# yijingru/KG_Instance_Segmentation

Measured on AMD Instinct MI355X. Metric: imgs/s (train fwd+bwd) at 512x512, higher is better.
Workload: dtype forward: f32-tolerance, hi + lo f16 planes (22 significant bits), 3 MFMA products / backward: f16 single planes, 1 MFMA product; f16 MFMA, fp32 accumulate; 1 GPU; KGnet train step fwd(dec+seg)+4xDetectionLossAll+SEG_loss+bwd+Adam, batch 8/GPU 3x512x512, 300 boxes/img, full HIP path; precision_policy=fp32, global_batch=8, parallelism=dp1, loss_readback=every step (train.py:156), grad_overflow=False

## Files before the change

### kg_instance_segmentation_amd/csrc/norm_pool.hip

```cpp
#include "kg_common.h"

struct RowsR { const bf16_t* p; int ld, P, ps; };
struct RowsW { bf16_t* p; int ld, P, ps; };
__device__ __forceinline__ void rd8(const RowsR& t, long r, int c, float (&v)[8]) { kg_load_planes8(t.p + r * t.ld + c, t.P, t.ps, v); }
__device__ __forceinline__ void wr8(const RowsW& t, long r, int c, float (&v)[8]) { kg_store_planes<8>(t.p + r * t.ld + c, t.P, t.ps, v, true); }
#define KG_PLANES(pl)                                                       \
    const kg_planes_t pp = kg_planes_or_default(pl);                        \
    KG_CHECK_ARG(kg_planes_ok(pp), "bad kg_planes_t (at most 3 planes, strides multiples of 8)")

__global__ void img_pack_kernel(const float* __restrict__ img, RowsW out, int N, int C, int HW) {
    long total = (long)N * HW;
    for (long i = blockIdx.x * (long)blockDim.x + threadIdx.x; i < total; i += (long)gridDim.x * blockDim.x) {
        long n = i / HW, p = i - n * HW;
        float v[8];
#pragma unroll
        for (int c = 0; c < 8; ++c) v[c] = c < C ? img[(n * C + c) * HW + p] : 0.f;
        wr8(out, i, 0, v);
    }
}
extern "C" int kg_img_pack(const float* img, void* out, int ldout, int N, int C, int H, int W, const kg_planes_t* planes, void* stream) {
    KG_CHECK_ARG(img && out && C <= 8 && ldout >= 8 && ldout % 8 == 0, "kg_img_pack: bad args");
    KG_PLANES(planes);
    long total = (long)N * H * W;
    int blocks = (int)((total + 255) / 256); if (blocks > 8192) blocks = 8192;
// ... 526 lines not shown
        }
        const float sy = (float)ih / (float)oh, sx = (float)iw / (float)ow;
        int ylo, yhi, xlo, xhi;
        bil_cand(iy, sy, oh, &ylo, &yhi); bil_cand(ix, sx, ow, &xlo, &xhi);
        float g[8];
#pragma unroll
        for (int e = 0; e < 8; ++e) g[e] = 0.f;
        for (int oy = ylo; oy <= yhi; ++oy) {
            int y0, y1; float ly;
            bil_src(oy, sy, ih, &y0, &y1, &ly);
            float wy = (y0 == iy ? 1.f - ly : 0.f) + (y1 == iy ? ly : 0.f);
            if (y0 != iy && y1 != iy) continue;
            for (int ox = xlo; ox <= xhi; ++ox) {
                int x0, x1; float lx;
                bil_src(ox, sx, iw, &x0, &x1, &lx);
                if (x0 != ix && x1 != ix) continue;
                float wx = (x0 == ix ? 1.f - lx : 0.f) + (x1 == ix ? lx : 0.f);
                float w = wy * wx;
                float ds[8];
                rd8(dy, out0 + (long)oy * ow + ox, c, ds);
#pragma unroll
                for (int e = 0; e < 8; ++e) g[e] += w * ds[e];
            }
        }
        if (mask) {
            const uint4 mv = *reinterpret_cast<const uint4*>(mask + p * ldmask + c);
            const bf16_t* ms = reinterpret_cast<const bf16_t*>(&mv);
#pragma unroll
            for (int e = 0; e < 8; ++e) g[e] = bf2f(ms[e]) > 0.f ? g[e] : 0.f;
        }
        wr8(dx, p, c, g);
    }
}
extern "C" int kg_bilinear_fwd(const void* x, int ldx, void* y, int ldy, int N, int IH, int IW, int OH, int OW, int C,
                               const int* boxdesc, const int* row2box, long total_out_rows, const kg_planes_t* planes, void* stream) {
    KG_CHECK_ARG(x && y && C % 8 == 0 && ldx % 8 == 0 && ldy % 8 == 0, "kg_bilinear_fwd: bad args");
    KG_PLANES(planes);
    long rows = boxdesc ? total_out_rows : (long)N * OH * OW;
    if (rows == 0) return KG_OK;
    long total = rows * (C / 8);
    static const int fast2x = getenv("KG_BILINEAR_2X") ? atoi(getenv("KG_BILINEAR_2X")) : 1;
    if (fast2x && !boxdesc && OH == 2 * IH && OW == 2 * IW && IH >= 2 && IW >= 2) {
        const long threads = (long)N * ((IH + BIL2_ROWS - 1) / BIL2_ROWS) * IW * (C / 8);
        int blocks2 = (int)((threads + 255) / 256); if (blocks2 > 65536) blocks2 = 65536;
        hipLaunchKernelGGL(bilinear2x_fwd_kernel, dim3(blocks2), dim3(256), 0, (hipStream_t)stream, RowsR{(const bf16_t*)x, ldx, pp.a_planes, pp.a_pstride},
                           RowsW{(bf16_t*)y, ldy, pp.y_planes, pp.y_pstride}, N, IH, IW, C / 8);
        KG_CHECK_LAUNCH("bilinear2x_fwd");
        return KG_OK;
    }
    int blocks = (int)((total + 255) / 256); if (blocks > 16384) blocks = 16384;
    hipLaunchKernelGGL(bilinear_fwd_kernel, dim3(blocks), dim3(256), 0, (hipStream_t)stream, RowsR{(const bf16_t*)x, ldx, pp.a_planes, pp.a_pstride},
                       RowsW{(bf16_t*)y, ldy, pp.y_planes, pp.y_pstride}, IH, IW, OH, OW, C / 8, rows, (const BilBox*)boxdesc, row2box);
    KG_CHECK_LAUNCH("bilinear_fwd");
    return KG_OK;
}
extern "C" int kg_bilinear_bwd(const void* dy, int lddy, void* dx, int lddx, int N, int IH, int IW, int OH, int OW, int C,
                               const int* boxdesc, const int* row2box, long total_in_rows, const void* mask, int ldmask,
                               const kg_planes_t* planes, void* stream) {
    KG_CHECK_ARG(dy && dx && C % 8 == 0 && lddy % 8 == 0 && lddx % 8 == 0 && (!mask || ldmask % 8 == 0), "kg_bilinear_bwd: bad args");
    KG_PLANES(planes);
    long rows = boxdesc ? total_in_rows : (long)N * IH * IW;
    if (rows == 0) return KG_OK;
    long total = rows * (C / 8);
    int blocks = (int)((total + 255) / 256); if (blocks > 16384) blocks = 16384;
    hipLaunchKernelGGL(bilinear_bwd_kernel, dim3(blocks), dim3(256), 0, (hipStream_t)stream, RowsR{(const bf16_t*)dy, lddy, pp.a_planes, pp.a_pstride},
                       RowsW{(bf16_t*)dx, lddx, pp.y_planes, pp.y_pstride}, IH, IW, OH, OW, C / 8, rows, (const BilBox*)boxdesc, row2box, (const bf16_t*)mask, ldmask);
    KG_CHECK_LAUNCH("bilinear_bwd");
    return KG_OK;
}

__global__ void add_rows_kernel(const RowsR a, const RowsR b,
                                const bf16_t* __restrict__ m, int ldm, const RowsW y, long M, int C8, const float* __restrict__ sc,
                                const float* __restrict__ sc2) {
    long total = M * C8;
    const float s = sc ? *sc * (sc2 ? *sc2 : 1.f) : 1.f;
    for (long i = blockIdx.x * (long)blockDim.x + threadIdx.x; i < total; i += (long)gridDim.x * blockDim.x) {
        long r; int c; kg_divmod(i, C8, &r, &c); c *= 8;
        float v[8];
        rd8(a, r, c, v);
        if (b.p) {
            float bs[8];
            rd8(b, r, c, bs);
#pragma unroll
            for (int e = 0; e < 8; ++e) v[e] += bs[e];
        }
        if (s != 1.f) {
#pragma unroll
            for (int e = 0; e < 8; ++e) v[e] *= s;
        }
        if (m) {
            uint4 mv = *reinterpret_cast<const uint4*>(m + r * ldm + c);
            const bf16_t* ms = (const bf16_t*)&mv;
#pragma unroll
            for (int e = 0; e < 8; ++e) v[e] = bf2f(ms[e]) > 0.f ? v[e] : 0.f;
        }
        wr8(y, r, c, v);
// ... 156 lines not shown
```

### kg_instance_segmentation_amd/csrc/conv_halo.hip

```cpp
#include "conv_args.h"
#include <type_traits>
#include <utility>
#include <stdlib.h>
#ifndef KG_HALO_SETPRIO
#define KG_HALO_SETPRIO 0
#endif
#ifndef KG_NARROW_V2
#define KG_NARROW_V2 1
#endif

__device__ uint4 kg_halo_zero_line[8];

struct HaloArgs {
    const bf16_t* x; const bf16_t* w; const float* bias;
    bf16_t* y; float* y_f32; const bf16_t* res; const bf16_t* mask;
    const int4* tiletab;
    int ntiles;
    int N, H, W, tiles_x, tiles_y;
    int cin_pad, ldx, Cout, ldy, ldres, ldmask, K, flip, relu, f32_C, f32_hw;
    int grp_chunks; const int* vmap; float* f32_b; float* f32_c;
    int xcd_map;
    int head_split;
    KMap km; int grp_C;
    float* stat_part;
    KgBStat bs;
    int kp_raw;
    int yP, yps, rP, rps;
    int walk3;
    const float* oscale;
    int prod_split; float* part;
    int ksplit; float* kpart;
    int nb2;
};

static void halo_set_walk(HaloArgs& a, int xP, int wP) {
    int xi[6], wj[6];
    const int nv = kg_plane_pairs(xP, wP, xi, wj);
    constexpr int on = 1;
    a.walk3 = on && nv == 3 && xi[0] == 0 && xi[1] == 1 && xi[2] == 0;
}

template <int KS, int WC, int WPX, int GM = 0, bool BSK = false>
__global__ __launch_bounds__(WC * WPX * 64) void conv_halo_kernel(const HaloArgs a) {
    constexpr int KSX = GM == 3 ? 1 : (GM == 4 ? 2 : KS);
    constexpr int PAD = KS / 2, TW = 4 * WPX, HWD = TW + KS - 1, HPIX = (16 + KS - 1) * HWD, TC = WC * 64, NT = WC * WPX * 64, T = KS * KSX;
    static_assert(GM < 3 || KS == 7, "the narrow variants are written for 7 x 7 kernels");
    constexpr int HALO_BYTES = HPIX * 128, WBUF_BYTES = TC * 128;
    constexpr bool GLW = KS == 7 && WC <= 2;
    constexpr int NSL = GLW ? 6 : 3;
    constexpr bool ASMRD = GLW && GM != 1;
    constexpr int WPT = TC * 8 / NT;
    extern __shared__ __attribute__((aligned(16))) unsigned char smem[];
    unsigned char* halo = smem;
    unsigned char* wbuf = smem + HALO_BYTES;

    const int tid = threadIdx.x, lane = tid & 63, wave = tid >> 6;
    const int wc = wave / WPX, wp = wave % WPX;
    const int lm = lane & 15, g = lane >> 4;
    int oy0, ox0, Hd, Wd;
    long rowbase;
    int bix = blockIdx.x, biy = blockIdx.y;
    if (a.xcd_map) {
        const int L = blockIdx.y * gridDim.x + blockIdx.x;
        const int xcd = L & 7, slot = L >> 3;
        biy = slot % gridDim.y;
        bix = xcd * (gridDim.x >> 3) + slot / gridDim.y;
    }
    if (a.tiletab) {
        const int4 tt = a.tiletab[bix];
        rowbase = tt.x; Hd = tt.y >> 16; Wd = tt.y & 0xffff; oy0 = tt.z >> 16; ox0 = tt.z & 0xffff;
    } else {
        int bt = bix;
        const int tx = bt % a.tiles_x; bt /= a.tiles_x;
        const int ty = bt % a.tiles_y; const int n = bt / a.tiles_y;
        oy0 = ty * 16; ox0 = tx * TW; Hd = a.H; Wd = a.W; rowbase = (long)n * a.H * a.W;
    }
    const int c0 = GM == 1 ? 0 : biy * TC;

    f32x4 acc[4][4];
#pragma unroll
    for (int i = 0; i < 4; ++i)
#pragma unroll
        for (int j = 0; j < 4; ++j) acc[i][j] = f32x4{0.f, 0.f, 0.f, 0.f};

    int a_off[4][2];
#pragma unroll
    for (int i = 0; i < 4; ++i) {
        const int r = wc * 64 + (lm >> 2) * 16 + i * 4 + (lm & 3);
        const int key = 2 * ((r >> 4) & 3) + ((r >> 1) & 1);
#pragma unroll
        for (int s = 0; s < 2; ++s) a_off[i][s] = r * 128 + (((4 * s + g) ^ key) * 16);
    }
    const int xb = (wp >> 2) * 16 + lm;
    int kb[KS][2];
#pragma unroll
    for (int kx = 0; kx < KS; ++kx) {
        if constexpr (GM >= 3) {
            if (kx < KSX) {
#pragma unroll
                for (int s = 0; s < 2; ++s) {
                    int kcol = GM == 3 ? 4 * s + g : 4 * kx + 2 * s + (g >> 1);
                    if (kcol > KS - 1) kcol = KS - 1;
                    const int slot = GM == 3 ? 0 : 1 + (g & 1);
                    const int fx = a.flip ? KS - 1 - kcol : kcol;
                    kb[kx][s] = (((wp & 3) * 4) * HWD + xb + fx) * 128 + ((slot ^ ((xb + fx) & 6)) * 16);
                }
            } else kb[kx][0] = kb[kx][1] = 0;
            continue;
        }
        const int fx = a.flip ? KS - 1 - kx : kx;
        const int key = (xb + fx) & 6;
#pragma unroll
        for (int s = 0; s < 2; ++s) kb[kx][s] = (((wp & 3) * 4) * HWD + xb) * 128 + (((4 * s + g) ^ key) * 16);
    }
    int ab[NSL][2];
#pragma unroll
    for (int q = 0; q < NSL; ++q)
#pragma unroll
        for (int s = 0; s < 2; ++s) ab[q][s] = q * WBUF_BYTES + a_off[0][s];

    int w_row[WPT], w_lds[WPT];
#pragma unroll
    for (int i = 0; i < WPT; ++i) {
        int e = tid + i * NT, r = e >> 3, c = e & 7;
        w_row[i] = r;
        w_lds[i] = r * 128 + ((c ^ (2 * ((r >> 4) & 3) + ((r >> 1) & 1))) * 16);
    }
    const int wc8 = (tid & 7) * 8;
    uint4 wreg[WPT];

    auto mma = [&](auto mk, const bf16x8 (&af)[4], const bf16x8 (&bfr)[4]) {
        constexpr int MK = decltype(mk)::value;
        if (KG_HALO_SETPRIO) __builtin_amdgcn_s_setprio(1);
#pragma unroll
        for (int i = 0; i < 4; ++i)
            if ((MK >> i) & 1) {
// ... 35 lines not shown
        else xo = a.km.xoff(cc);
        if (!stage) {
        } else if (KS == 3) {
            constexpr int HPT = (HPIX * 8 + NT - 1) / NT;
            uint4 hreg[HPT];
#pragma unroll
            for (int q = 0; q < HPT; ++q) {
                const int e = tid + q * NT;
                const int p = e >> 3, c = e & 7;
                const int hy = p / HWD, hx = p - hy * HWD;
                const int iy = oy0 + hy - PAD, ix = ox0 + hx - PAD;
                uint4 v = make_uint4(0, 0, 0, 0);
                if (e < HPIX * 8 && (unsigned)iy < (unsigned)Hd && (unsigned)ix < (unsigned)Wd)
                    v = *reinterpret_cast<const uint4*>(a.x + (rowbase + (long)iy * Wd + ix) * a.ldx + xo + c * 8);
                hreg[q] = v;
            }
#pragma unroll
            for (int q = 0; q < HPT; ++q) {
                const int e = tid + q * NT;
                const int p = e >> 3, c = e & 7;
                const int hx = p % HWD;
                if (e < HPIX * 8) *reinterpret_cast<uint4*>(halo + p * 128 + ((c ^ (hx & 6)) * 16)) = hreg[q];
            }
        } else
        {
            constexpr int HPT = (HPIX * 8 + NT - 1) / NT;
            const int wave_u = __builtin_amdgcn_readfirstlane(wave);
#pragma unroll 1
            for (int q = 0; q < HPT; ++q) {
                const int e = tid + q * NT;
                if (e < HPIX * 8) {
                    const int p = e >> 3, cs = e & 7;
                    const int hy = p / HWD, hx = p - hy * HWD;
                    const int c = cs ^ (hx & 6);
                    const int iy = oy0 + hy - PAD, ix = ox0 + hx - PAD;
                    const bf16_t* src = reinterpret_cast<const bf16_t*>(kg_halo_zero_line) + c * 8;
                    if ((unsigned)iy < (unsigned)Hd && (unsigned)ix < (unsigned)Wd)
                        src = a.x + (rowbase + (long)iy * Wd + ix) * a.ldx + xo + c * 8;
                    __builtin_amdgcn_global_load_lds((const __attribute__((address_space(1))) void*)src,
                                                     (__attribute__((address_space(3))) void*)(halo + (q * NT + wave_u * 64) * 16), 16, 0, 0);
                }
            }
        }
        if constexpr (GM == 1) {
            const int head_n = cc / a.grp_chunks;
            if (head_n < 2) {
                constexpr int ROWB = 7 * 2048;
                const int wave_n = __builtin_amdgcn_readfirstlane(wave);
#if KG_NARROW_V2
                const bf16_t* nsrc[2];
#pragma unroll
                for (int k = 0; k < 2; ++k) {
                    const int e = tid + k * 512, kyl = e >> 7, rho = (e >> 3) & 15, sl = e & 7;
                    const int r = 16 * (rho >> 2) + 4 * head_n + (rho & 3);
                    const int key = 2 * (rho >> 2) + ((rho >> 1) & 1);
                    nsrc[k] = a.w + (long)r * a.K + (long)(kyl * KS) * a.cin_pad + cc * 64 + ((sl ^ key) * 8);
                }
                auto nload = [&](int kx) {
                    unsigned char* dst = wbuf + (kx % 3) * ROWB + wave_n * 1024;
                    const long ro = (long)kx * a.cin_pad;
                    __builtin_amdgcn_global_load_lds((const __attribute__((address_space(1))) void*)(nsrc[0] + ro),
                                                     (__attribute__((address_space(3))) void*)dst, 16, 0, 0);
                    if (wave_n < 6)
                        __builtin_amdgcn_global_load_lds((const __attribute__((address_space(1))) void*)(nsrc[1] + ro),
                                                         (__attribute__((address_space(3))) void*)(dst + 8192), 16, 0, 0);
                };
                nload(0); nload(1);
// ... 128 lines not shown
#pragma unroll
            for (int i = 0; i < WPT; ++i) *reinterpret_cast<uint4*>(wbuf + slot_bytes + w_lds[i]) = wreg[i];
        };
        const bf16_t* wsrc[WPT];
        auto wglds = [&](int slot_bytes) {
#pragma unroll
            for (int i = 0; i < WPT; ++i) {
                __builtin_amdgcn_global_load_lds((const __attribute__((address_space(1))) void*)wsrc[i],
                                                 (__attribute__((address_space(3))) void*)(wbuf + slot_bytes + (i * NT + __builtin_amdgcn_readfirstlane(wave) * 64) * 16), 16, 0, 0);
                wsrc[i] += a.cin_pad;
            }
        };
        auto wait_newest = [&]() {
            if constexpr (WPT == 1) asm volatile("s_waitcnt vmcnt(1)" ::: "memory");
            else asm volatile("s_waitcnt vmcnt(2)" ::: "memory");
        };
        static_assert(!GLW || WPT <= 2, "counted waits are written for 1 or 2 loads per slice");
        if constexpr (GLW) {
#pragma unroll
            for (int i = 0; i < WPT; ++i) {
                const int e = tid + i * NT, r = e >> 3, cs = e & 7;
                wsrc[i] = a.w + (long)(c0 + r) * a.K + cc * 64 + (cs ^ (2 * ((r >> 4) & 3) + ((r >> 1) & 1))) * 8;
            }
            wglds(0); wglds(WBUF_BYTES); wglds(2 * WBUF_BYTES); wglds(3 * WBUF_BYTES);
            wait_newest();
            __builtin_amdgcn_s_barrier();
            asm volatile("" ::: "memory");
        } else {
            wload(0); wstore(0);
            if (T > 1) { wload(1); wstore(1); }
            if (T > 2) wload(2);
            __syncthreads();
        }
        bf16x8 a0[4], b0[4], a1[4], b1[4];
        if constexpr (ASMRD) {
#pragma unroll
            for (int i = 0; i < 4; ++i) { a0[i] = bf16x8{0, 0, 0, 0, 0, 0, 0, 0}; a1[i] = a0[i]; }
        }
        const unsigned lds0 = lds_addr(smem);
        int abr[NSL][2];
        int sbr[NSL];
#pragma unroll
        for (int q = 0; q < NSL; ++q) { abr[q][0] = ab[q][0]; abr[q][1] = ab[q][1]; sbr[q] = q * WBUF_BYTES; }
        int tapb = a.flip ? ((KS - 1) * HWD + (GM >= 3 ? 0 : KS - 1)) * 128 : 0;
        const int sx = a.flip ? -128 : 128, sy = a.flip ? -HWD * 128 : HWD * 128;
        auto ldA = [&](auto mk, bf16x8 (&af)[4], int base) {
            constexpr int MK = decltype(mk)::value;
            if constexpr (ASMRD) {
                const unsigned ad = lds0 + HALO_BYTES + base;
                if (MK & 1) lds_rd128<0>(af[0], ad);
                if (MK & 2) lds_rd128<512>(af[1], ad);
                if (MK & 4) lds_rd128<1024>(af[2], ad);
                if (MK & 8) lds_rd128<1536>(af[3], ad);
            } else {
#pragma unroll
                for (int i = 0; i < 4; ++i)
                    if ((MK >> i) & 1) af[i] = *reinterpret_cast<const bf16x8*>(wbuf + base + i * 512);
            }
        };
        auto ldB = [&](bf16x8 (&bfr)[4], int tb, int kbv) {
            if constexpr (ASMRD) {
                const unsigned ad = lds0 + tb + kbv;
                lds_rd128<0>(bfr[0], ad); lds_rd128<HWD * 128>(bfr[1], ad); lds_rd128<2 * HWD * 128>(bfr[2], ad); lds_rd128<3 * HWD * 128>(bfr[3], ad);
            } else {
                const unsigned char* hb = halo + tb + kbv;
#pragma unroll
// ... 581 lines not shown
        }
    }
    if (!bsk) {
        hipLaunchKernelGGL((conv_halo_kernel<KS, WC, WPX, GM>), grid, dim3(WC * WPX * 64), smem, st, a);
        KG_KNAME(kname, "conv_halo_kernel<%d, %d, %d, %d>", KS, WC, WPX, GM);
        kg_note_kernel(kname);
    }
    KG_CHECK_LAUNCH("conv_halo");
    if (a.ksplit > 1) {
        hipLaunchKernelGGL((conv_halo_finish_kernel<WC, WPX>), dim3(grid.x, grid.y), dim3(WC * WPX * 64), 0, st, a);
        KG_CHECK_LAUNCH("conv_halo_finish");
    }
    return KG_OK;
}

extern "C" int kg_conv2d_halo(const void* x, const void* w, const float* bias, void* y, float* y_f32, const void* res,
                              const void* mask, int N, int H, int W, int cin_pad, int ldx, int Cout, int ldy, int ldres,
                              int ldmask, int K, int KS, int flip, int relu, int f32_C, int wc, const int* tiletab,
                              int ntiles, int total_rows, const kg_planes_t* planes, void* stream) {
    HaloArgs a;
    memset(&a, 0, sizeof(a));
    const kg_planes_t pp = kg_planes_or_default(planes);
    KG_CHECK_ARG(kg_planes_ok(pp), "kg_conv2d_halo: bad kg_planes_t");
    int segs_[3];
    const int vplanes = kg_kmap_segs(pp.a_planes, pp.w_planes, segs_);
    a.km = kg_make_kmap(cin_pad, 64, pp.a_planes, pp.a_pstride, pp.w_planes);
    halo_set_walk(a, pp.a_planes, pp.w_planes);
    a.yP = pp.y_planes; a.yps = pp.y_pstride; a.rP = pp.b_planes; a.rps = pp.b_pstride; a.oscale = pp.oscale;
    KG_CHECK_ARG(!(y_f32 && (res || mask)), "kg_conv2d_halo: fp32 exports take no residual / mask");
    KG_CHECK_ARG(x && w && (y || y_f32), "kg_conv2d_halo: null pointer");
    KG_CHECK_ARG(KS == 3 || KS == 7, "kg_conv2d_halo: kernel size must be 3 or 7");
    KG_CHECK_ARG(cin_pad % 64 == 0 && ldx % 8 == 0, "kg_conv2d_halo: cin_pad must be a multiple of 64 (got %d)", cin_pad);
    const int narrow = (wc >> 9) & 3;
    KG_CHECK_ARG(narrow == 0 || (narrow <= 2 && KS == 7 && cin_pad == 64 && vplanes == 1 && (wc & 255) <= 1 && !tiletab && y && !y_f32),
                 "kg_conv2d_halo: the narrow variants take one 64-channel single-plane dense input and a rows output");
    KG_CHECK_ARG(K >= (narrow ? 7 * narrow * 64 : KS * KS * cin_pad * vplanes), "kg_conv2d_halo: K too small");
    KG_CHECK_ARG((tiletab && ntiles > 0 && Cout > 0) || (N > 0 && H > 0 && W > 0 && Cout > 0), "kg_conv2d_halo: empty problem");
    a.x = (const bf16_t*)x; a.w = (const bf16_t*)w; a.bias = bias; a.y = (bf16_t*)y; a.y_f32 = y_f32;
    a.res = (const bf16_t*)res; a.mask = (const bf16_t*)mask;
    a.N = N; a.H = H; a.W = W; a.tiles_x = kg_cdiv(W, 16); a.tiles_y = kg_cdiv(H, 16);
    a.cin_pad = cin_pad * vplanes; a.ldx = ldx; a.Cout = Cout; a.ldy = ldy; a.ldres = ldres; a.ldmask = ldmask; a.K = K;
    a.flip = flip; a.relu = relu; a.f32_C = f32_C; a.tiletab = (const int4*)tiletab; a.ntiles = ntiles; a.f32_hw = total_rows;
    {
        const KgConvStats& cs = kg_conv_stats();
        const bool want = cs.bs.x ? (flip && KS == 3 && wc <= 1 && !tiletab && Cout % 64 == 0) : (!res && !mask && !relu && !flip);
        if (y && !y_f32 && want && cs.part && cs.nb == 0)
            a.stat_part = cs.part;
    }
    const int k1skip = (wc >> 8) & 1; wc &= 255;
    if (wc == 0) wc = 1;
    hipStream_t st = (hipStream_t)stream;
    if (KS == 7) {
        switch (wc) {
            case 1:
                if (narrow == 1) return launch_halo<7, 1, 8, 3>(a, st);
                if (narrow == 2) return launch_halo<7, 1, 8, 4>(a, st);
                return k1skip ? launch_halo<7, 1, 8, 2>(a, st) : launch_halo<7, 1, 8>(a, st);
            case 2: return launch_halo<7, 2, 4>(a, st);
            case 3: return launch_halo<7, 3, 4>(a, st);
        }
    } else {
        switch (wc) {
            case 1: return launch_halo<3, 1, 8>(a, st);
            case 2: return launch_halo<3, 2, 4>(a, st);
            case 3: return launch_halo<3, 3, 4>(a, st);
        }
    }
    kg_set_error("kg_conv2d_halo: bad wc %d", wc);
    return KG_ERR_ARG;
}

__global__ __launch_bounds__(256) void heads2_finish_kernel(const float* __restrict__ part, long per_z, int Z, int N, long hw, float* __restrict__ kp,
                                                            float* __restrict__ sh, float* __restrict__ md, int kp_raw) {
    for (long i = (long)blockIdx.x * 256 + threadIdx.x; i < per_z; i += (long)gridDim.x * 256) {
        double acc = 0.;
        for (int z = 0; z < Z; ++z) acc += (double)part[z * per_z + i];
        const float v = (float)acc;
        const long pix = i % hw, q = i / hw;
        const int ch = (int)(q % 55); const long n = q / 55;
        if (ch < 5) kp[(n * 5 + ch) * hw + pix] = kp_raw ? v : 1.f / (1.f + expf(-v));
        else if (ch < 15) sh[(n * 10 + ch - 5) * hw + pix] = v;
        else md[(n * 40 + ch - 15) * hw + pix] = v;
    }
}

extern "C" int kg_conv2d_halo_heads2(const void* x, const void* w, const float* bias64, const int* vmap, float* kp, float* sh,
                                     float* md, int N, int H, int W, int C, int ldx, int K, int kp_sigmoid, const kg_planes_t* planes, void* stream) {
    HaloArgs a;
    memset(&a, 0, sizeof(a));
// ... 68 lines not shown
```

### kg_instance_segmentation_amd/engine.py

```python
import os

import torch

from . import arch, ops
from .ops import BF16, PT, PackedWeight

PRECISIONS = {
    "fp32": (2, 2, 2, 2, 1),
    "fp32b2": (2, 2, 2, 2, 2),
    "half": (1, 1, 1, 1, 1),
    "halfmix": (2, 1, 1, 1, 1),
    "fp32bf": (3, 3, 3, 3, 2),
    "fp32bf_full": (3, 3, 3, 3, 3),
    "fp32bf_w1d1": (3, 3, 3, 3, 2, 1, 1),
    "fp32bf_b1": (3, 3, 3, 3, 1),
    "trunk2": (2, 2, 1, 1, 1), "mixed": (2, 1, 1, 1, 1), "bf16": (1, 1, 1, 1, 1),
}
HALF_POLICIES = ("fp32", "fp32b2", "half", "halfmix")
DEFAULT_PRECISION = "fp32"
PRE = [0]
NARROW_HEADS_DGRAD = int(os.environ.get("KG_NARROW_HEADS_DGRAD", "2"))
BN_BWD_STATS = True


def default_precision():
    p = os.environ.get("KG_PRECISION", DEFAULT_PRECISION)
    if p not in PRECISIONS:
        raise ValueError(f"KG_PRECISION must be one of {sorted(PRECISIONS)} (got {p!r})")
    return p


def trunc(t, P):
    if isinstance(t, PT):
        return t if t.P <= P else PT(t.t, P, t.ps)
    return t


class Var:
    __slots__ = ("t", "C", "relu", "grad", "masked", "pending", "pmasked", "req", "parent", "c0", "gP", "bn_part", "boundary", "gsc",
                 "uses", "ngot", "bn_in", "bstat")
    ENG = None

    def __init__(self, t, C, relu=False, req=True, parent=None, c0=0, gP=None):
        self.t = t if isinstance(t, PT) else PT(t)
        self.C, self.relu, self.req = C, relu, req
        self.gP = self.t.P if gP is None else gP
        self.grad, self.masked = None, True
        self.pending, self.pmasked = None, True
        self.parent, self.c0 = parent, c0
        self.boundary = False
        self.uses, self.ngot = 0, 0
        self.bn_in = None
        self.bstat = None
        self.gsc = None
# ... 588 lines not shown
        self._phase("end")
        if self.nbt:
            torch._foreach_add_(self.nbt, 1)
            self.nbt = []
        if self.stats_written:
            ops.PARAM_EPOCH[0] += 1
        self.feats, self.dims, self.N, self.maps = feats, dims, N, maps
        for fv in feats:
            fv.uses += 1 << 20
        feats[1].boundary = True
        return maps, feats, dims

    HEAD_OFF = (0, 8, 24)
    HEAD_PAD = (8, 16, 40)

    def heads2_tables(self, dev):
        t = getattr(self, "_heads2", None)
        if t is None or t["vmap"].device != dev:
            rows, vmap = ops.heads2_layout()
            vm = torch.tensor(vmap, dtype=torch.int32)
            t = {"rows": [torch.tensor(r, dtype=torch.int32, device=dev) for r in rows], "vmap": vm.to(dev),
                 "bias_idx": torch.where(vm < 0, torch.full_like(vm, 55), vm).long().to(dev),
                 "zero1": torch.zeros(1, dtype=torch.float32, device=dev)}
            self._heads2 = t
        return t

    def prepare_heads2(self, lvl, C, dev, train):
        self.heads2_seen[lvl] = (C, dev)
        key = f"heads_c{lvl}.2F"
        ent = self.fusedT.get(key)
        if self.fast_stamp is not None and ent is not None and ent[0][:3] == self.fast_stamp and ent[1].buf.device == dev:
            entT = self.fusedT.get(f"heads_c{lvl}.2T") if train else None
            if not train or (entT is not None and entT[0][:3] == self.fast_stamp and entT[1].buf.device == dev):
                return ent[1], ent[2], (entT[1], entT[2]) if train else None
        ph = self.ph
        specs = [self.spec(f"{h}_head_c{lvl}.2", C, co, 7, 1, 3, P=ph) for h, co in arch.HEADS]
        ws = [self.P(s.names[0] + ".weight") for s in specs]
        bs = [self.P(s.names[0] + ".bias") for s in specs]
        ver = self.stamp + tuple(t._version for t in ws + bs) + tuple(t.data_ptr() for t in ws + bs)
        if ent is None or ent[0] != ver or ent[1].buf.device != dev:
            lay = self.heads2_tables(dev)
            pwF = ent[1] if ent is not None and ent[1].buf.device == dev else PackedWeight(64, 49, C, dev, xP=ph, wP=ph, groups=3, dtype=self.dt)
            for k, w in enumerate(ws):
                pwF.pack_rows(w.detach(), lay["rows"][k], group=k)
            bias64 = torch.cat([b.detach() for b in bs] + [lay["zero1"]])[lay["bias_idx"]]
            self.fusedT[key] = (ver, pwF, bias64)
        _, pwF, bias64 = self.fusedT[key]
        pwT = None
        if train:
            key = f"heads_c{lvl}.2T"
            ent = self.fusedT.get(key)
            ver = self.stamp + tuple(w._version for w in ws) + tuple(w.data_ptr() for w in ws)
            if ent is None or ent[0] != ver or ent[1].buf.device != dev:
                gph = min(ph, self.pg)
                reuse = ent is not None and ent[1].buf.device == dev
                pwT = ent[1] if reuse else PackedWeight(3 * C, 49, 64, dev, xP=gph, wP=min(gph, self.pdw), dtype=self.dt)
                narrow = NARROW_HEADS_DGRAD and gph == 1 and min(gph, self.pdw) == 1
                pwN = None
                if narrow:
                    pwN = ent[2] if reuse and ent[2] is not None else (PackedWeight(C, 7, 64, dev, dtype=self.dt), PackedWeight(C, 14, 64, dev, dtype=self.dt))
                    pwN[0].pack_narrow(ws[0].detach(), 8)
                    pwN[1].pack_narrow(ws[1].detach(), 16)
                for k, w in enumerate(ws):
                    if narrow and k < 2:
                        continue
                    pwT.pack(w.detach(), row0=k * C, c0=self.HEAD_OFF[k], transposed=True)
                self.fusedT[key] = (ver, pwT, pwN)
            pwT = (self.fusedT[key][1], self.fusedT[key][2])
        return pwF, bias64, pwT

    def heads_second(self, hid, lvl, C, N, H, W):
        dev = hid.t.device
        train = self.tape is not None
        specs = [self.spec(f"{h}_head_c{lvl}.2", C, co, 7, 1, 3, P=self.ph) for h, co in arch.HEADS]
        pwF, bias64, pwTN = self.prepare_heads2(lvl, C, dev, train)
        pwT, pwN = pwTN if pwTN is not None else (None, None)
        outs = [torch.empty(N, co, H, W, dtype=torch.float32, device=dev) for _, co in arch.HEADS]
        ops.conv_halo_heads2(hid.t, pwF, bias64, self.heads2_tables(dev)["vmap"], outs[0], outs[1], outs[2], N, H, W, C,
                             kp_sigmoid=not self.raw_kp_logits)
        if self.keep_kp_logits:
            side = [torch.empty_like(o) for o in outs]
            ops.conv_halo_heads2(hid.t, pwF, bias64, self.heads2_tables(dev)["vmap"], side[0], side[1], side[2], N, H, W, C, kp_sigmoid=False)
            self.kp_logits[lvl] = side[0]
        slot = {"grad": None}
        self.head_slots.append((slot, lvl, N, H, W))
        wreq = [train and self.trainable((s.names[0] + ".weight", s.names[0] + ".bias")) for s in specs]
        if train and (hid.req or any(wreq)):
            geom = (N * H * W, H, W, H, W, 7, 7, 1, 3)

            def bwd():
                g = slot["grad"]
                if g is None:
                    return
                for k, ((h, co), s) in enumerate(zip(arch.HEADS, specs)):
                    if not wreq[k]:
                        continue
                    gk = g.cols(self.HEAD_OFF[k], self.HEAD_OFF[k] + self.HEAD_PAD[k])
                    w = self.P(s.names[0] + ".weight")
                    gw = self.new_grad(s.names[0] + ".weight", w)
                    db = self.new_grad(s.names[0] + ".bias", self.P(s.names[0] + ".bias"))
                    ops.conv_wgrad(trunc(hid.t, min(hid.gP, self.pw)).cols(k * C, (k + 1) * C), trunc(gk, self.pw), C, co, geom, [(gw, 0, co)], N=N, bias_out=db)
                    self.param_grads[s.names[0] + ".weight"] = gw
                    self.param_grads[s.names[0] + ".bias"] = db
                if not hid.req:
                    return
                dh = ops.alloc_pt(hid.rows, 3 * C, hid.gP, dev, dtype=self.dt)
                if pwN is not None and g.P == 1 and NARROW_HEADS_DGRAD >= 2 and dh.P == 1:
                    ops.conv7_narrow(g, pwN[0], C, N, H, W, dh.cols(0, C), mask=hid.t.hi()[:, :C], chan_lo=0, chan_slot=8, algo_cin=5)
                    ops.conv7_narrow(g, pwN[1], C, N, H, W, dh.cols(C, 2 * C), mask=hid.t.hi()[:, C:2 * C], chan_lo=8, chan_slot=16, algo_cin=10)
                elif pwN is not None and g.P == 1:
                    ops.conv_halo(g, pwN[0], C, N, H, W, 7, y=dh.cols(0, C), mask=hid.t.hi()[:, :C], flip=True, narrow=8, algo_cin=5)
                    ops.conv_halo(g, pwN[1], C, N, H, W, 7, y=dh.cols(C, 2 * C), mask=hid.t.hi()[:, C:2 * C], flip=True, narrow=16, algo_cin=10)
                else:
                    ops.conv_halo(g, pwT, 2 * C, N, H, W, 7, y=dh.cols(0, 2 * C), mask=hid.t.hi()[:, :2 * C], flip=True, k1skip=True, algo_cin=7.5)
                ops.conv_halo(g, pwT.rows_from(2 * C), C, N, H, W, 7, y=dh.cols(2 * C, 3 * C), mask=hid.t.hi()[:, 2 * C:], flip=True, algo_cin=40)
                hid.add_grad(dh, masked=True)
            self.tape.append(bwd)
        return outs

    def export_feats(self):
        outs = []
        for fv, (h, w) in zip(self.feats, self.dims):
            o = torch.empty(fv.rows, fv.C, dtype=torch.float32, device=fv.t.device)
            ops.planes_to_f32(fv.t, fv.C, o)
            outs.append(o.view(self.N, h, w, fv.C).permute(0, 3, 1, 2))
        return outs

    def backward_dec(self, map_grads, feat_grads, gscale=None):
        if gscale is not None:
            self.gscale = gscale
            Var.ENG = self
        gsc = self.gscale[0:1] if self.gscale is not None else None
        if self.grad_store is not None:
            self.grad_store.dense_backward_started()
        for (slot, lvl, N, Hh, Wh) in self.head_slots:
            gs = map_grads[3 * lvl:3 * lvl + 3]
            if all(g is None for g in gs):
                continue
            dev = self.maps[3 * lvl].device
            packed = ops.alloc_pt(N * Hh * Wh, 64, min(self.ph, self.pg), dev, dtype=self.dt)
            if all(g is not None for g in gs) and self.HEAD_OFF == (0, 8, 24) and sum(self.HEAD_PAD) == 64:
                ops.grad_pack3([g.contiguous().float() for g in gs], self.maps[3 * lvl], packed, N, [co for _, co in arch.HEADS], Hh, Wh, self.HEAD_PAD, scale=gsc)
                slot["grad"] = packed
                continue
            for k, g in enumerate(gs):
                co = arch.HEADS[k][1]
                view = packed.cols(self.HEAD_OFF[k], self.HEAD_OFF[k] + self.HEAD_PAD[k])
                if g is None:
# ... 50 lines not shown
```

### kg_instance_segmentation_amd/ops.py

```python
import functools
import math
import os

import torch

from . import _lib
from ._lib import c_int, c_long, c_float, c_double, ptr, stream_ptr

BF16 = torch.bfloat16
F16 = torch.float16
_scratch = {}
PARAM_EPOCH = [0]


def scratch_f32(nfloats, dev, tag="default"):
    key = (str(dev), tag)
    t = _scratch.get(key)
    if t is None or t.numel() < nfloats:
        t = torch.empty(max(int(nfloats), 1 << 16), dtype=torch.float32, device=dev)
        _scratch[key] = t
    return t


class WgradReduceQueue:
# ... 246 lines not shown
    if PACKQ16.jobs:
        PACKQ16.flush(hold)


def launch_held_packs():
    if PACKQ.pending is not None:
        PACKQ.launch_pending()
    if PACKQ16.pending is not None:
        PACKQ16.launch_pending()


class PackedWeight:

    def __init__(self, rows, taps, cin_pad, dev, xP=1, wP=1, groups=1, dtype=BF16):
        self.rows, self.taps, self.cin_pad, self.xP, self.wP, self.groups = rows, taps, cin_pad, xP, wP, groups
        self.vp = vplanes(xP, wP)
        self.tap_stride = groups * self.vp * cin_pad
        self.K = round_up((round_up(taps, 4) if cin_pad == 8 else taps) * self.tap_stride, 64)
        self.buf = torch.zeros(round_up(rows, 384), self.K, dtype=dtype, device=dev)

    def pack(self, w, row0=0, c0=0, transposed=False):
        Cout, Cin, KH, KW = w.shape
        assert w.dtype == torch.float32 and w.is_contiguous()
        assert self.groups == 1
        if PACKQ.defer:
            (PACKQ16 if fmt_of(self) else PACKQ).add(w, self, row0, c0, transposed, None)
            return
        _lib.call("kg_pack_weight", ptr(w), ptr(self.buf), Cout, Cin, KH, KW, self.K, self.cin_pad, row0, c0,
                  1 if transposed else 0, self.xP, self.wP, stream_ptr(), fmt=fmt_of(self))


    def pack_narrow(self, w, chan_slot, row0=0):
        Cout, Cin, KH, KW = w.shape
        assert w.dtype == torch.float32 and w.is_contiguous() and KH == KW == 7 and Cout <= chan_slot and self.xP == self.wP == 1
        assert self.cin_pad == 64 and self.K >= 7 * 8 * chan_slot
        if PACKQ.defer:
            (PACKQ16 if fmt_of(self) else PACKQ).add(w, self, row0, 0, True, None, tap_stride=chan_slot, tap_pitch=8, cin_pad=chan_slot)
            return
        _lib.call("kg_pack_weight_narrow", ptr(w), ptr(self.buf), Cout, Cin, KH, KW, self.K, row0, 0, chan_slot, 8, stream_ptr(), fmt=fmt_of(self))

    def rows_from(self, r0):
        v = PackedWeight.__new__(PackedWeight)
        v.rows, v.taps, v.cin_pad, v.K, v.buf = self.rows - r0, self.taps, self.cin_pad, self.K, self.buf[r0:]
        v.xP, v.wP, v.groups, v.vp, v.tap_stride = self.xP, self.wP, self.groups, self.vp, self.tap_stride
        return v

    def pack_rows(self, w, rowmap, group=0):
        Cout, Cin, KH, KW = w.shape
        assert w.dtype == torch.float32 and w.is_contiguous() and rowmap.dtype == torch.int32 and rowmap.numel() == Cout
        c0 = group * self.vp * self.cin_pad
        if PACKQ.defer:
            (PACKQ16 if fmt_of(self) else PACKQ).add(w, self, 0, c0, False, rowmap, self.tap_stride)
            return
        _lib.call("kg_pack_weight_rows", ptr(w), ptr(self.buf), Cout, Cin, KH, KW, self.K, self.cin_pad, ptr(rowmap), c0,
                  self.xP, self.wP, self.tap_stride, stream_ptr(), fmt=fmt_of(self))


def heads2_layout():
    grp = [[16 * q + 4 * i + r for q in range(4) for r in range(4)] for i in range(4)]
    rows = [grp[0][:5], grp[1][:10], grp[2] + grp[3] + grp[0][5:13]]
    vmap = [-1] * 64
    base = (0, 5, 15)
    for h in range(3):
        for c, v in enumerate(rows[h]):
            vmap[v] = base[h] + c
    return rows, vmap

# ... 35 lines not shown
IM2COL_WGRAD = True


HALO_WC = 0


USE_WS = True


def conv_halo(x, pw, cout, N, H, W, KS, y=None, y_f32=None, bias=None, res=None, mask=None, relu=False, flip=False, wc=0,
              tiletab=None, total_rows=0, k1skip=False, algo_cin=None, tiletab16=None, oscale=None, tiletab8=None, narrow=0):
    flush_packs()
    assert nplanes(x)[0] == pw.xP, (nplanes(x), pw.xP)
    if (USE_WS and KS == 3 and pw.cin_pad == 64 and cout == 64 and pw.xP == 2 and pw.wP == 2 and y is not None and y_f32 is None and res is None
            and mask is None and not flip and oscale is None and wc == 0 and HALO_WC == 0 and (tiletab is None or tiletab8 is not None)
            and nplanes(y)[0] <= 2 and not conv_stats_armed()):
        _lib.call("kg_conv3x3_ws", ptr(_rows(x)), ptr(pw.buf), ptr(bias), ptr(base(y)), N, H, W, ld(x), ld(y), pw.K, 1 if relu else 0,
                  ptr(tiletab8), tiletab8.shape[0] if tiletab8 is not None else 0, pl(a=x, y=y, w=pw.wP), stream_ptr(), fmt=fmt_of(x))
        return
    planes = pl(a=x, b=res, y=y, w=pw.wP, oscale=oscale)
    x, y, res, mask = base(x), base(y), base(res), base(mask)
    if (USE_C3 and planes is None and KS == 3 and pw.cin_pad == 64 and y is not None and y_f32 is None and wc == 0 and HALO_WC == 0
            and (tiletab is None or tiletab16 is not None)):
        flush_packs()
        _lib.call("kg_conv3x3_c64", ptr(_rows(x)), ptr(pw.buf), ptr(bias), ptr(y), ptr(res), ptr(mask), N, H, W, ld(x), cout, ld(y),
                  ld(res) if res is not None else 0, ld(mask) if mask is not None else 0, pw.K, 1 if flip else 0, 1 if relu else 0,
                  ptr(tiletab16), tiletab16.shape[0] if tiletab16 is not None else 0, stream_ptr(), fmt=fmt_of(x))
        return
    wc = wc or HALO_WC
    if k1skip:
        assert KS == 7 and wc in (0, 1)
        wc = 1 | 256
    if narrow:
        assert KS == 7 and wc in (0, 1) and flip and narrow in (8, 16) and planes is None and tiletab is None and y is not None and y_f32 is None
        wc = 1 | (512 if narrow == 8 else 1024)
    f32_C = 0
    if y_f32 is not None:
        f32_C = y_f32.shape[1] if y_f32.dim() == 4 else 1
    _lib.call("kg_conv2d_halo", ptr(_rows(x)), ptr(pw.buf), ptr(bias), ptr(y), ptr(y_f32), ptr(res), ptr(mask), N, H, W,
              pw.cin_pad, ld(x), cout, ld(y) if y is not None else 0, ld(res) if res is not None else 0,
              ld(mask) if mask is not None else 0, pw.K, KS, 1 if flip else 0, 1 if relu else 0, f32_C, wc, ptr(tiletab),
              tiletab.shape[0] if tiletab is not None else 0, total_rows, planes, stream_ptr(), fmt=fmt_of(x))


USE_1X1 = True
GATHER_1X1 = True


def conv1x1(x, pw, cout, y, bias=None, res=None, mask=None, relu=False):
    flush_packs()
    assert pw.vp == 1 and all(nplanes(t)[0] == 1 for t in (x, y, res))
    x, y, res, mask = base(x), base(y), base(res), base(mask)
    _lib.call("kg_conv1x1", ptr(_rows(x)), ptr(pw.buf), ptr(bias), ptr(_rows(y)), ptr(res), ptr(mask), c_long(x.shape[0]),
              pw.cin_pad, pw.K, ld(x), cout, ld(y), ld(res) if res is not None else 0, ld(mask) if mask is not None else 0,
              1 if relu else 0, stream_ptr(), fmt=fmt_of(x))


def can_1x1(x, pw, KH, stride, pad, y, y_f32, res=None):
    if pw.vp > 1 or any(nplanes(t)[0] > 1 for t in (x, y, res)):
        return False
    if GATHER_1X1 and pw.cin_pad >= 192 and pw.rows > 64:
        return False
    return (USE_1X1 and KH == 1 and stride == 1 and pad == 0 and y is not None and y_f32 is None and pw.cin_pad % 64 == 0
            and 64 <= pw.cin_pad <= 1024 and x.shape[1] >= pw.cin_pad and y.shape[0] == x.shape[0])


CONV_TINY_WGS = 96
CONV_TINY_TILES = 384
# ... 372 lines not shown
```

Measured before the change: 129.4 imgs/s.

## Add specialized 2x bilinear backward kernel with sliding row window over strips

Adds a dedicated backward kernel for exact 2x bilinear upsampling on single-plane gradients. Each thread walks a vertical strip of input rows and keeps a 4x4 window of output-gradient chunks in registers, reusing two rows between steps instead of rescanning candidate output pixels. The strip height is chosen so enough threads remain for occupancy. Odd zero-weight loads at the borders appear to mimic the generic kernel's summation order, which adds code complexity and some extra loads.

```diff
diff --git a/kg_instance_segmentation_amd/csrc/norm_pool.hip b/kg_instance_segmentation_amd/csrc/norm_pool.hip
--- a/kg_instance_segmentation_amd/csrc/norm_pool.hip
+++ b/kg_instance_segmentation_amd/csrc/norm_pool.hip
@@ -582,6 +582,76 @@
         wr8(dx, p, c, g);
     }
 }
+struct BilChunk {
+    uint4 q;
+    __device__ __forceinline__ void load(const RowsR& t, long r, int c) { q = *reinterpret_cast<const uint4*>(t.p + r * t.ld + c); }
+    __device__ __forceinline__ void get(float (&v)[8]) const {
+        const bf16_t* s = reinterpret_cast<const bf16_t*>(&q);
+#pragma unroll
+        for (int e = 0; e < 8; ++e) v[e] = bf2f(s[e]);
+    }
+};
+__global__ __launch_bounds__(256) void bilinear2x_bwd_kernel(const RowsR dy, const RowsW dx, int N, int IH, int IW, int C8, int strip_rows,
+                                                             const bf16_t* __restrict__ mask, int ldmask) {
+    const long per_img = (long)IW * C8;
+    const int strips = (IH + strip_rows - 1) / strip_rows;
+    const long total = (long)N * strips * per_img;
+    const int OH = 2 * IH, OW = 2 * IW;
+    for (long t = blockIdx.x * (long)blockDim.x + threadIdx.x; t < total; t += (long)gridDim.x * blockDim.x) {
+        long q; int c; kg_divmod(t, C8, &q, &c); c *= 8;
+        int j; long q2; kg_divmod(q, IW, &q2, &j);
+        int strip; long n; kg_divmod(q2, strips, &n, &strip);
+        const int i0 = strip * strip_rows, i1 = i0 + strip_rows < IH ? i0 + strip_rows : IH;
+        const long in0 = n * IH * IW, out0 = n * OH * OW;
+        const int ox0 = j > 0 ? 2 * j - 1 : 0, ox3 = j < IW - 1 ? 2 * j + 2 : OW - 1;
+        const float wx1 = j == 0 ? 1.f : 0.75f, wx2 = j == IW - 1 ? 1.f : 0.75f;
+        BilChunk win[4][4];
+        auto load_row = [&](BilChunk (&r)[4], int oy) {
+            const long b = out0 + (long)oy * OW;
+            r[0].load(dy, b + ox0, c); r[1].load(dy, b + 2 * j, c); r[2].load(dy, b + 2 * j + 1, c); r[3].load(dy, b + ox3, c);
+        };
+        load_row(win[0], i0 > 0 ? 2 * i0 - 1 : 0);
+        load_row(win[1], 2 * i0);
+        for (int i = i0; i < i1; ++i) {
+            load_row(win[2], 2 * i + 1);
+            load_row(win[3], i < IH - 1 ? 2 * i + 2 : OH - 1);
+            float g[8];
+#pragma unroll
+            for (int e = 0; e < 8; ++e) g[e] = 0.f;
+            auto acc = [&](const BilChunk& ch, float w) {
+                float d[8];
+                ch.get(d);
+#pragma unroll
+                for (int e = 0; e < 8; ++e) g[e] = __builtin_fmaf(w, d[e], g[e]);
+            };
+            auto row = [&](const BilChunk (&r)[4], int oy, float wy) {
+                if (j == 1) { BilChunk z; z.load(dy, out0 + (long)oy * OW, c); acc(z, wy * 0.f); }
+                if (j > 0) acc(r[0], wy * 0.25f);
+                acc(r[1], wy * wx1);
+                acc(r[2], wy * wx2);
+                if (j < IW - 1) acc(r[3], wy * 0.25f);
+            };
+            if (i == 1) {
+                const int cols[5] = {0, ox0, 2 * j, 2 * j + 1, ox3};
+                for (int k = j == 1 ? 0 : j > 0 ? 1 : 2; k < (j < IW - 1 ? 5 : 4); ++k) { BilChunk z; z.load(dy, out0 + cols[k], c); acc(z, 0.f); }
+            }
+            if (i > 0) row(win[0], 2 * i - 1, 0.25f);
+            row(win[1], 2 * i, i == 0 ? 1.f : 0.75f);
+            row(win[2], 2 * i + 1, i == IH - 1 ? 1.f : 0.75f);
+            if (i < IH - 1) row(win[3], 2 * i + 2, 0.25f);
+            const long p = in0 + (long)i * IW + j;
+            if (mask) {
+                const uint4 mv = *reinterpret_cast<const uint4*>(mask + p * ldmask + c);
+                const bf16_t* ms = reinterpret_cast<const bf16_t*>(&mv);
+#pragma unroll
+                for (int e = 0; e < 8; ++e) g[e] = bf2f(ms[e]) > 0.f ? g[e] : 0.f;
+            }
+            wr8(dx, p, c, g);
+#pragma unroll
+            for (int k = 0; k < 4; ++k) { win[0][k] = win[2][k]; win[1][k] = win[3][k]; }
+        }
+    }
+}
 extern "C" int kg_bilinear_fwd(const void* x, int ldx, void* y, int ldy, int N, int IH, int IW, int OH, int OW, int C,
                                const int* boxdesc, const int* row2box, long total_out_rows, const kg_planes_t* planes, void* stream) {
     KG_CHECK_ARG(x && y && C % 8 == 0 && ldx % 8 == 0 && ldy % 8 == 0, "kg_bilinear_fwd: bad args");
@@ -612,6 +682,17 @@
     long rows = boxdesc ? total_in_rows : (long)N * IH * IW;
     if (rows == 0) return KG_OK;
     long total = rows * (C / 8);
+    static const int fast2x = getenv("KG_BILINEAR_2X_BWD") ? atoi(getenv("KG_BILINEAR_2X_BWD")) : 1;
+    if (fast2x && !boxdesc && pp.a_planes == 1 && OH == 2 * IH && OW == 2 * IW && IH >= 2 && IW >= 2) {
+        int strip_rows = 8;
+        while (strip_rows > 2 && (long)N * ((IH + strip_rows - 1) / strip_rows) * IW * (C / 8) < 256L * 1024) strip_rows /= 2;
+        const long threads = (long)N * ((IH + strip_rows - 1) / strip_rows) * IW * (C / 8);
+        int blocks2 = (int)((threads + 255) / 256); if (blocks2 > 65536) blocks2 = 65536;
+        hipLaunchKernelGGL(bilinear2x_bwd_kernel, dim3(blocks2), dim3(256), 0, (hipStream_t)stream, RowsR{(const bf16_t*)dy, lddy, pp.a_planes, pp.a_pstride},
+                           RowsW{(bf16_t*)dx, lddx, pp.y_planes, pp.y_pstride}, N, IH, IW, C / 8, strip_rows, (const bf16_t*)mask, ldmask);
+        KG_CHECK_LAUNCH("bilinear2x_bwd");
+        return KG_OK;
+    }
     int blocks = (int)((total + 255) / 256); if (blocks > 16384) blocks = 16384;
     hipLaunchKernelGGL(bilinear_bwd_kernel, dim3(blocks), dim3(256), 0, (hipStream_t)stream, RowsR{(const bf16_t*)dy, lddy, pp.a_planes, pp.a_pstride},
                        RowsW{(bf16_t*)dx, lddx, pp.y_planes, pp.y_pstride}, IH, IW, OH, OW, C / 8, rows, (const BilBox*)boxdesc, row2box, (const bf16_t*)mask, ldmask);
```

Result: no change. 129.0 imgs/s (median of 2 runs) (-0.3%).

## Add narrow 40-channel dgrad variant for third head's 7x7 backward conv

Applied to the files above, without the earlier changes.

Adds a GM==5 halo-conv variant that packs the third head's transposed weights with 40-channel tap slots, so its 7x7 data-gradient conv covers 35 K-chunks instead of 49 full 64-channel taps. It maps the kernel columns and slot indices onto the packed layout and runs a dedicated unrolled MFMA loop with its own weight prefetch and barriers. The variant is turned on by default through a new environment switch, cutting padded MFMA work for that backward conv. It adds a specialised code path whose slot and remapping logic must line up exactly with the packing, and its changed synchronisation pattern could cost occupancy or correctness.

```diff
diff --git a/kg_instance_segmentation_amd/csrc/conv_halo.hip b/kg_instance_segmentation_amd/csrc/conv_halo.hip
--- a/kg_instance_segmentation_amd/csrc/conv_halo.hip
+++ b/kg_instance_segmentation_amd/csrc/conv_halo.hip
@@ -42,7 +42,7 @@
 
 template <int KS, int WC, int WPX, int GM = 0, bool BSK = false>
 __global__ __launch_bounds__(WC * WPX * 64) void conv_halo_kernel(const HaloArgs a) {
-    constexpr int KSX = GM == 3 ? 1 : (GM == 4 ? 2 : KS);
+    constexpr int KSX = GM == 3 ? 1 : (GM == 4 ? 2 : (GM == 5 ? 5 : KS));
     constexpr int PAD = KS / 2, TW = 4 * WPX, HWD = TW + KS - 1, HPIX = (16 + KS - 1) * HWD, TC = WC * 64, NT = WC * WPX * 64, T = KS * KSX;
     static_assert(GM < 3 || KS == 7, "the narrow variants are written for 7 x 7 kernels");
     constexpr int HALO_BYTES = HPIX * 128, WBUF_BYTES = TC * 128;
@@ -100,8 +100,14 @@
 #pragma unroll
                 for (int s = 0; s < 2; ++s) {
                     int kcol = GM == 3 ? 4 * s + g : 4 * kx + 2 * s + (g >> 1);
+                    int slot = GM == 3 ? 0 : 1 + (g & 1);
+                    if constexpr (GM == 5) {
+                        const int q = 8 * kx + 4 * s + g;
+                        kcol = q / 5;
+                        slot = 3 + q - 5 * kcol;
+                        if (q > 34 || (slot == 3 && (g & 1))) slot = 2;
+                    }
                     if (kcol > KS - 1) kcol = KS - 1;
-                    const int slot = GM == 3 ? 0 : 1 + (g & 1);
                     const int fx = a.flip ? KS - 1 - kcol : kcol;
                     kb[kx][s] = (((wp & 3) * 4) * HWD + xb + fx) * 128 + ((slot ^ ((xb + fx) & 6)) * 16);
                 }
@@ -203,7 +209,8 @@
                 if (e < HPIX * 8) {
                     const int p = e >> 3, cs = e & 7;
                     const int hy = p / HWD, hx = p - hy * HWD;
-                    const int c = cs ^ (hx & 6);
+                    int c = cs ^ (hx & 6);
+                    if constexpr (GM == 5) { if (c == 2) c = 3; }
                     const int iy = oy0 + hy - PAD, ix = ox0 + hx - PAD;
                     const bf16_t* src = reinterpret_cast<const bf16_t*>(kg_halo_zero_line) + c * 8;
                     if ((unsigned)iy < (unsigned)Hd && (unsigned)ix < (unsigned)Wd)
@@ -398,6 +405,38 @@
             if (T > 2) wload(2);
             __syncthreads();
         }
+        if constexpr (GM == 5) {
+            constexpr int NU = 9 * KS;
+            const unsigned ldsb = lds_addr(smem);
+            const unsigned wad[2] = {ldsb + HALO_BYTES + (unsigned)a_off[0][0], ldsb + HALO_BYTES + (unsigned)a_off[0][1]};
+            bf16x8 fa[2][4], fb[2][4];
+            auto rd = [&](auto uc) {
+                constexpr int U = decltype(uc)::value, KY = U / 9, V = (U % 9) >> 1, S = (U % 9) & 1, B = U & 1, SL = ((KY * KSX + V) % NSL) * WBUF_BYTES;
+                lds_rd128<SL>(fa[B][0], wad[S]); lds_rd128<SL + 512>(fa[B][1], wad[S]); lds_rd128<SL + 1024>(fa[B][2], wad[S]); lds_rd128<SL + 1536>(fa[B][3], wad[S]);
+                const unsigned ad = ldsb + (a.flip ? KS - 1 - KY : KY) * (HWD * 128) + kb[V][S];
+                lds_rd128<0>(fb[B][0], ad); lds_rd128<HWD * 128>(fb[B][1], ad); lds_rd128<2 * HWD * 128>(fb[B][2], ad); lds_rd128<3 * HWD * 128>(fb[B][3], ad);
+            };
+            auto kstep = [&](auto uc) {
+                constexpr int U = decltype(uc)::value, KY = U / 9, V = (U % 9) >> 1, S = (U % 9) & 1, B = U & 1, TT = KY * KSX + V;
+                constexpr bool first = S == 0, last = S == 1 || V == KSX - 1;
+                if constexpr (first && !(TT & 1)) {
+                    if constexpr (TT + 4 < T) wglds(((TT + 4) % NSL) * WBUF_BYTES);
+                    if constexpr (TT + 5 < T) wglds(((TT + 5) % NSL) * WBUF_BYTES);
+                }
+                if constexpr (U + 1 < NU) { rd(std::integral_constant<int, U + 1>{}); lgkm_wait<8>(fa[B], fb[B]); }
+                else lgkm_wait<0>(fa[B], fb[B]);
+                mma(std::integral_constant<int, 15>{}, fa[B], fb[B]);
+                if constexpr (last && (TT & 1) && TT + 1 < T) {
+                    if constexpr (TT + 4 < T) wait_newest();
+                    else asm volatile("s_waitcnt vmcnt(0)" ::: "memory");
+                    __builtin_amdgcn_s_barrier();
+                    asm volatile("" ::: "memory");
+                }
+            };
+            rd(std::integral_constant<int, 0>{});
+            [&]<int... Us>(std::integer_sequence<int, Us...>) { (kstep(std::integral_constant<int, Us>{}), ...); }(std::make_integer_sequence<int, NU>{});
+            continue;
+        }
         bf16x8 a0[4], b0[4], a1[4], b1[4];
         if constexpr (ASMRD) {
 #pragma unroll
@@ -1045,9 +1084,9 @@
     KG_CHECK_ARG(KS == 3 || KS == 7, "kg_conv2d_halo: kernel size must be 3 or 7");
     KG_CHECK_ARG(cin_pad % 64 == 0 && ldx % 8 == 0, "kg_conv2d_halo: cin_pad must be a multiple of 64 (got %d)", cin_pad);
     const int narrow = (wc >> 9) & 3;
-    KG_CHECK_ARG(narrow == 0 || (narrow <= 2 && KS == 7 && cin_pad == 64 && vplanes == 1 && (wc & 255) <= 1 && !tiletab && y && !y_f32),
+    KG_CHECK_ARG(narrow == 0 || (KS == 7 && cin_pad == 64 && vplanes == 1 && (wc & 255) <= 1 && !tiletab && y && !y_f32),
                  "kg_conv2d_halo: the narrow variants take one 64-channel single-plane dense input and a rows output");
-    KG_CHECK_ARG(K >= (narrow ? 7 * narrow * 64 : KS * KS * cin_pad * vplanes), "kg_conv2d_halo: K too small");
+    KG_CHECK_ARG(K >= (narrow == 3 ? 35 * 64 : narrow ? 7 * narrow * 64 : KS * KS * cin_pad * vplanes), "kg_conv2d_halo: K too small");
     KG_CHECK_ARG((tiletab && ntiles > 0 && Cout > 0) || (N > 0 && H > 0 && W > 0 && Cout > 0), "kg_conv2d_halo: empty problem");
     a.x = (const bf16_t*)x; a.w = (const bf16_t*)w; a.bias = bias; a.y = (bf16_t*)y; a.y_f32 = y_f32;
     a.res = (const bf16_t*)res; a.mask = (const bf16_t*)mask;
@@ -1068,6 +1107,7 @@
             case 1:
                 if (narrow == 1) return launch_halo<7, 1, 8, 3>(a, st);
                 if (narrow == 2) return launch_halo<7, 1, 8, 4>(a, st);
+                if (narrow == 3) return launch_halo<7, 1, 8, 5>(a, st);
                 return k1skip ? launch_halo<7, 1, 8, 2>(a, st) : launch_halo<7, 1, 8>(a, st);
             case 2: return launch_halo<7, 2, 4>(a, st);
             case 3: return launch_halo<7, 3, 4>(a, st);
diff --git a/kg_instance_segmentation_amd/engine.py b/kg_instance_segmentation_amd/engine.py
--- a/kg_instance_segmentation_amd/engine.py
+++ b/kg_instance_segmentation_amd/engine.py
@@ -20,6 +20,7 @@
 DEFAULT_PRECISION = "fp32"
 PRE = [0]
 NARROW_HEADS_DGRAD = int(os.environ.get("KG_NARROW_HEADS_DGRAD", "2"))
+MID_HEADS_DGRAD = int(os.environ.get("KG_MID_HEADS_DGRAD", "1"))
 BN_BWD_STATS = True
 
 
@@ -674,7 +675,7 @@
         if self.fast_stamp is not None and ent is not None and ent[0][:3] == self.fast_stamp and ent[1].buf.device == dev:
             entT = self.fusedT.get(f"heads_c{lvl}.2T") if train else None
             if not train or (entT is not None and entT[0][:3] == self.fast_stamp and entT[1].buf.device == dev):
-                return ent[1], ent[2], (entT[1], entT[2]) if train else None
+                return ent[1], ent[2], (entT[1], entT[2], entT[3]) if train else None
         ph = self.ph
         specs = [self.spec(f"{h}_head_c{lvl}.2", C, co, 7, 1, 3, P=ph) for h, co in arch.HEADS]
         ws = [self.P(s.names[0] + ".weight") for s in specs]
@@ -703,12 +704,17 @@
                     pwN = ent[2] if reuse and ent[2] is not None else (PackedWeight(C, 7, 64, dev, dtype=self.dt), PackedWeight(C, 14, 64, dev, dtype=self.dt))
                     pwN[0].pack_narrow(ws[0].detach(), 8)
                     pwN[1].pack_narrow(ws[1].detach(), 16)
+                mid = MID_HEADS_DGRAD and gph == 1 and min(gph, self.pdw) == 1
+                pwM = None
+                if mid:
+                    pwM = ent[3] if reuse and ent[3] is not None else PackedWeight(C, 35, 64, dev, dtype=self.dt)
+                    pwM.pack_narrow(ws[2].detach(), 40)
                 for k, w in enumerate(ws):
-                    if narrow and k < 2:
+                    if (narrow and k < 2) or (mid and k == 2):
                         continue
                     pwT.pack(w.detach(), row0=k * C, c0=self.HEAD_OFF[k], transposed=True)
-                self.fusedT[key] = (ver, pwT, pwN)
-            pwT = (self.fusedT[key][1], self.fusedT[key][2])
+                self.fusedT[key] = (ver, pwT, pwN, pwM)
+            pwT = self.fusedT[key][1:4]
         return pwF, bias64, pwT
 
     def heads_second(self, hid, lvl, C, N, H, W):
@@ -716,7 +722,7 @@
         train = self.tape is not None
         specs = [self.spec(f"{h}_head_c{lvl}.2", C, co, 7, 1, 3, P=self.ph) for h, co in arch.HEADS]
         pwF, bias64, pwTN = self.prepare_heads2(lvl, C, dev, train)
-        pwT, pwN = pwTN if pwTN is not None else (None, None)
+        pwT, pwN, pwM = pwTN if pwTN is not None else (None, None, None)
         outs = [torch.empty(N, co, H, W, dtype=torch.float32, device=dev) for _, co in arch.HEADS]
         ops.conv_halo_heads2(hid.t, pwF, bias64, self.heads2_tables(dev)["vmap"], outs[0], outs[1], outs[2], N, H, W, C,
                              kp_sigmoid=not self.raw_kp_logits)
@@ -755,7 +761,10 @@
                     ops.conv_halo(g, pwN[1], C, N, H, W, 7, y=dh.cols(C, 2 * C), mask=hid.t.hi()[:, C:2 * C], flip=True, narrow=16, algo_cin=10)
                 else:
                     ops.conv_halo(g, pwT, 2 * C, N, H, W, 7, y=dh.cols(0, 2 * C), mask=hid.t.hi()[:, :2 * C], flip=True, k1skip=True, algo_cin=7.5)
-                ops.conv_halo(g, pwT.rows_from(2 * C), C, N, H, W, 7, y=dh.cols(2 * C, 3 * C), mask=hid.t.hi()[:, 2 * C:], flip=True, algo_cin=40)
+                if pwM is not None:
+                    ops.conv_halo(g, pwM, C, N, H, W, 7, y=dh.cols(2 * C, 3 * C), mask=hid.t.hi()[:, 2 * C:], flip=True, narrow=40, algo_cin=40)
+                else:
+                    ops.conv_halo(g, pwT.rows_from(2 * C), C, N, H, W, 7, y=dh.cols(2 * C, 3 * C), mask=hid.t.hi()[:, 2 * C:], flip=True, algo_cin=40)
                 hid.add_grad(dh, masked=True)
             self.tape.append(bwd)
         return outs
diff --git a/kg_instance_segmentation_amd/ops.py b/kg_instance_segmentation_amd/ops.py
--- a/kg_instance_segmentation_amd/ops.py
+++ b/kg_instance_segmentation_amd/ops.py
@@ -302,7 +302,7 @@
 
     def pack_narrow(self, w, chan_slot, row0=0):
         Cout, Cin, KH, KW = w.shape
-        assert w.dtype == torch.float32 and w.is_contiguous() and KH == KW == 7 and Cout <= chan_slot and self.xP == self.wP == 1
+        assert w.dtype == torch.float32 and w.is_contiguous() and KH == KW == 7 and Cout <= chan_slot and self.xP == self.wP == 1 and chan_slot in (8, 16, 40)
         assert self.cin_pad == 64 and self.K >= 7 * 8 * chan_slot
         if PACKQ.defer:
             (PACKQ16 if fmt_of(self) else PACKQ).add(w, self, row0, 0, True, None, tap_stride=chan_slot, tap_pitch=8, cin_pad=chan_slot)
@@ -404,8 +404,8 @@
         assert KS == 7 and wc in (0, 1)
         wc = 1 | 256
     if narrow:
-        assert KS == 7 and wc in (0, 1) and flip and narrow in (8, 16) and planes is None and tiletab is None and y is not None and y_f32 is None
-        wc = 1 | (512 if narrow == 8 else 1024)
+        assert KS == 7 and wc in (0, 1) and flip and narrow in (8, 16, 40) and planes is None and tiletab is None and y is not None and y_f32 is None
+        wc = 1 | {8: 512, 16: 1024, 40: 1536}[narrow]
     f32_C = 0
     if y_f32 is not None:
         f32_C = y_f32.shape[1] if y_f32.dim() == 4 else 1
```

Result: no change. 129.6 imgs/s before, 130.6 imgs/s after (median of 6 runs) (+0.7%).
